# lithium0003/findtextCenterNet

Hardware: AMD Instinct MI355X
Metric: 768x768 images/s (detector fwd+NMS) (higher is better)
Workload: dtype bf16; 1 GPU; BASELINE configs[1]: batch=8/GPU synthetic 768x768x3 uniform-noise tiles, full EfficientNetV2-XL detector forward + NMS + GPU peak decode/100-d gather; global_batch=8, tile=768x768x3, weights=deterministic seed 0 (random-init), parallelism=dp1

## Files before the change

### findtextcenternet_amd/csrc/mbconv_slice.hip

```cpp
#include "conv_igemm_impl.h"

namespace {
using namespace convimpl;

struct MbsP {
    const void* x;
    const void* we;
    const float* be;
    const float* wd;
    const float* bd;
    void* out;
    float* sums;
    const float* w1;
    float* hpart;
    int B, H, W, K, C, S;
    int R, nb;
    int kblock;
    unsigned img_bytes;
    float inv_hw;
    unsigned long long* tl;
};

constexpr int MS_NT = 512;
constexpr int MS_MAXPX = 576;
constexpr int MS_XS = MS_MAXPX * 64;
constexpr int MS_NSTAGE = 3;
constexpr int MS_MAXSLOT = 601;
constexpr int MS_R = 6;
template <int NCT> struct MsGeom {
    static constexpr int CC = NCT * 32;
    static constexpr int CQN = CC / 4;
    static constexpr int NPL = MS_NT / CQN;
    static constexpr int STAGE = MS_XS + CC * 64;
    static constexpr int PITCH = CC * 2 + 8;
    static constexpr int IMG = MS_MAXSLOT * PITCH, RING = MS_NSTAGE * STAGE;
    static constexpr int CONST = ((IMG > RING ? IMG : RING) + 15) / 16 * 16;
    static constexpr int LDS = CONST + 10 * CC * 4;
    static constexpr int NPIECE = 36 + CC / 16;
    static constexpr int NW6 = NPIECE - 40;
    static_assert(LDS <= 160 * 1024 && NPIECE > 40 && NPIECE <= 48, "");
};

__device__ __forceinline__ f32x4 mfma16x16(bf16x8 a, bf16x8 b, f32x4 c) { return __builtin_amdgcn_mfma_f32_16x16x32_bf16(a, b, c, 0, 0, 0); }
__device__ __forceinline__ f32x4 mfma16x16(f16x8 a, f16x8 b, f32x4 c) { return __builtin_amdgcn_mfma_f32_16x16x32_f16(a, b, c, 0, 0, 0); }

template <typename T> struct Raw4;
template <> struct Raw4<__bf16> { using type = bf16x4; };
template <> struct Raw4<_Float16> { using type = f16x4; };
template <typename V> __device__ __forceinline__ f32x4 widen4(V v) { return f32x4{(float)v[0], (float)v[1], (float)v[2], (float)v[3]}; }
template <int N> struct MsInt { static constexpr int value = N; };

constexpr int MS_GENERAL = 0, MS_MAP24 = 1, MS_BAND48 = 2;

template <typename T, int FORM, int NCT = 4>
__global__ __launch_bounds__(MS_NT, 2) void mbconv_slice_kernel(const MbsP p) {
    constexpr bool FAST = FORM == MS_MAP24;
    using GM = MsGeom<NCT>;
    constexpr int MS_CC = GM::CC, MS_STAGE = GM::STAGE, MS_PITCH = GM::PITCH, MS_CONST = GM::CONST, CQN = GM::CQN, NPL = GM::NPL;
    extern __shared__ __attribute__((aligned(16))) unsigned char smem_raw[];
    const int t = threadIdx.x;
    const int lane = t & 63;
    const int wave = __builtin_amdgcn_readfirstlane(t >> 6);
    const int l15 = lane & 15, lq = lane >> 4;
    const int bid = blockIdx.x;
    const int b = bid % p.B;
    const int rest = bid / p.B;
    const int band = FAST ? 0 : rest % p.nb, sl = FAST ? rest : rest / p.nb;
    const int c0 = sl * MS_CC;
    const int W = FAST ? 24 : FORM == MS_BAND48 ? 48 : p.W;
    const int y0 = FAST ? 0 : band * p.R, y1 = FAST ? 24 : min(p.H, y0 + p.R);
    const int ylo = FAST ? 0 : max(0, y0 - 1), yhi = FAST ? 24 : min(p.H, y1 + 1);
    const int H = yhi - ylo;
    const int M = H * W;
    const int W1 = W + 1;
    const int Mfull = p.H * W;

    const unsigned xbase = (unsigned)ylo * W * (p.kblock ? 64u : (unsigned)p.K * 2u);
    const __amdgpu_buffer_rsrc_t rx = __builtin_amdgcn_make_buffer_rsrc(const_cast<char*>(static_cast<const char*>(p.x) + (size_t)b * p.img_bytes + xbase), 0,
                                                                        p.img_bytes - xbase, 0x00020000);
    const __amdgpu_buffer_rsrc_t rwe = __builtin_amdgcn_make_buffer_rsrc(const_cast<char*>(static_cast<const char*>(p.we) + (size_t)c0 * p.K * 2), 0,
                                                                         (unsigned)(MS_CC * p.K * 2), 0x00020000);

    constexpr int NLMAX = 6;
    int s_off[NLMAX];
#pragma unroll
    for (int i = 0; i < NLMAX; ++i) {
        const int q = (i * 8 + wave) * 64 + lane;
        const bool isx = q < MS_MAXPX * 4;
        const int row = isx ? (q >> 2) : ((q - MS_MAXPX * 4) >> 2);
        const int kc = (q & 3) ^ (((row >> 3) & 1) * 3);
        const int rowb = (isx && p.kblock) ? 64 : p.K * 2;
        s_off[i] = (!isx || row < M) ? row * rowb + kc * 16 : OOB;
    }
    const int xstep = p.kblock ? Mfull * 64 : 64;
    auto issue_piece = [&](int i, int step, int bufoff) {
        const int q0 = (i * 8 + wave) * 64;
        if (i < 5 || wave < GM::NW6) {
            lds_void_t* dst = (lds_void_t*)(smem_raw + bufoff + q0 * 16);
            if (q0 < MS_MAXPX * 4) glds16(rx, dst, s_off[i], step * xstep);
            else glds16(rwe, dst, s_off[i], step * 64);
        }
    };

    const int chw = wave & 1, pg = wave >> 1;
    f32x4 acc[NCT][9];
#pragma unroll
    for (int i = 0; i < NCT; ++i) {
        const f32x4 bi = *reinterpret_cast<const f32x4*>(p.be + c0 + chw * (MS_CC / 2) + i * 16 + 4 * lq);
#pragma unroll
        for (int j = 0; j < 9; ++j) acc[i][j] = bi;
    }
    if (t < 10 * CQN) {
        const int row = t / CQN, ch = (t - row * CQN) * 4;
        const f32x4 v = *reinterpret_cast<const f32x4*>(row < 9 ? p.wd + (long)row * p.C + c0 + ch : p.bd + c0 + ch);
        *reinterpret_cast<f32x4*>(smem_raw + MS_CONST + t * 16) = v;
    }

    using FragT = typename Frag<T>::type;
    const int swz = ((lq ^ (((l15 >> 3) & 1) * 3)) << 4);
    const int offA = MS_XS + (chw * (MS_CC / 2) + l15) * 64 + swz;
    const int offB = (pg * 144 + l15) * 64 + swz;
    const int nk = p.K >> 5;
    const bool tl_on = p.tl && t == 0;
    unsigned long long* tl = p.tl + (size_t)blockIdx.x * 32;
    if (tl_on) tl[0] = __builtin_amdgcn_s_memtime();
#pragma unroll
    for (int i = 0; i < NLMAX; ++i) issue_piece(i, 0, 0);
    if (nk > 1) {
#pragma unroll
        for (int i = 0; i < NLMAX; ++i) issue_piece(i, 1, MS_STAGE);
    }
    int cur_off = 0, iss_off = 2 * MS_STAGE;
    unsigned long long tw = 0, tw0 = 0;
    for (int it = 0; it < nk; ++it) {
        const unsigned long long ta = tl_on ? __builtin_amdgcn_s_memtime() : 0;
        if (it + 1 >= nk) wait_vmcnt<0>();
        else if (wave < GM::NW6) wait_vmcnt<6>();
        else wait_vmcnt<5>();
        wg_barrier();
        if (tl_on) { const unsigned long long d = __builtin_amdgcn_s_memtime() - ta; tw += d; if (it == 0) tw0 = d; if (it < 24) tl[8 + it] = ta; }
        const unsigned char* base = smem_raw + cur_off;
        const bool more = it + 2 < nk;
        FragT af[NCT];
#pragma unroll
        for (int i = 0; i < NCT; ++i) af[i] = *reinterpret_cast<const FragT*>(base + offA + i * 1024);
        FragT bq[3];
#pragma unroll
        for (int j = 0; j < 3; ++j) bq[j] = *reinterpret_cast<const FragT*>(base + offB + j * 1024);
#pragma unroll
        for (int j = 0; j < 9; ++j) {
            const FragT bcur = bq[j % 3];
            if (j + 3 < 9) bq[j % 3] = *reinterpret_cast<const FragT*>(base + offB + (j + 3) * 1024);
#pragma unroll
            for (int i = 0; i < NCT; ++i) acc[i][j] = mfma16x16(af[i], bcur, acc[i][j]);
            constexpr int piece_after[9] = {0, 1, -1, 2, 3, -1, 4, 5, -1};
            if (piece_after[j] >= 0 && more) issue_piece(piece_after[j], it + 2, iss_off);
            __builtin_amdgcn_sched_barrier(0);
        }
        iss_off = iss_off + MS_STAGE == MS_NSTAGE * MS_STAGE ? 0 : iss_off + MS_STAGE;
        cur_off = cur_off + MS_STAGE == MS_NSTAGE * MS_STAGE ? 0 : cur_off + MS_STAGE;
    }
    wg_barrier();
    if (tl_on) { tl[1] = __builtin_amdgcn_s_memtime(); tl[5] = tw; tl[6] = tw0; }

    for (int idx = t; idx < (H + 1) * CQN; idx += MS_NT) {
        const u32x2 z = {0u, 0u};
        *reinterpret_cast<u32x2*>(smem_raw + ((idx / CQN) * W1) * MS_PITCH + (idx % CQN) * 8) = z;
    }
#pragma unroll
    for (int j = 0; j < 9; ++j) {
        const int m = pg * 144 + j * 16 + l15;
        if (m < M) {
            const int y = m / W;
            unsigned char* row = smem_raw + (m + y + 1) * MS_PITCH + (chw * (MS_CC / 2) + 4 * lq) * 2;
#pragma unroll
            for (int i = 0; i < NCT; ++i) store4<T>(reinterpret_cast<T*>(row + i * 32), act_silu_fast4(acc[i][j]));
        }
    }
    __syncthreads();
    if (tl_on) tl[2] = __builtin_amdgcn_s_memtime();

    const int pl = t / CQN, cq = t - pl * CQN;
    const bool dw_on = pl < NPL;
    const int c = c0 + cq * 4;
    constexpr int NU = (FTC_MBHEAD_MAX_SQUEEZE + NPL - 1) / NPL;
    f32x4 w1r[NU];
    auto load_w1 = [&]() {
#pragma unroll
        for (int i = 0; i < NU; ++i) {
            const int su = pl + NPL * i;
            w1r[i] = (dw_on && su < p.S) ? *reinterpret_cast<const f32x4*>(p.w1 + (size_t)su * p.C + c) : f32x4{0.f, 0.f, 0.f, 0.f};
        }
    };
    if (p.hpart) load_w1();
    f32x4 wv[9];
#pragma unroll
    for (int k = 0; k < 9; ++k) wv[k] = *reinterpret_cast<const f32x4*>(smem_raw + MS_CONST + k * (MS_CC * 4) + cq * 16);
    const f32x4 bv = *reinterpret_cast<const f32x4*>(smem_raw + MS_CONST + 9 * (MS_CC * 4) + cq * 16);
    const int yo = y0 - ylo, yend = y1 - ylo;
    const int nsr = (yend - yo + MS_R - 1) / MS_R;
    const int nstrips = nsr * W;
    f32x4 sum = {0.f, 0.f, 0.f, 0.f};
    T* outp = reinterpret_cast<T*>(p.out) + ((size_t)b * Mfull + (size_t)ylo * W) * p.C + c;
    const unsigned char* zslot = smem_raw + cq * 8;
    using R4 = typename Raw4<T>::type;
    auto run_strips = [&](auto nr_c, int s, const int lim) __attribute__((always_inline)) {
        constexpr int NR = decltype(nr_c)::value;
        for (; s < lim; s += NPL) {
            const int sr = s / W, x = s - sr * W;
            const int oy0 = yo + sr * MS_R;
            const unsigned char* base0 = smem_raw + ((oy0 - 1) * W1 + x) * MS_PITCH + cq * 8;
            const unsigned char* base1 = base0 + 7 * W1 * MS_PITCH;
            R4 win[(NR + 2) * 3];
#pragma unroll
            for (int r = 0; r < NR + 2; ++r) {
                const bool rok = r == 0 ? oy0 > 0 : r == NR + 1 ? oy0 + NR < H : true;
                const unsigned char* rp = (r < 7 ? base0 + r * W1 * MS_PITCH : base1 + (r - 7) * W1 * MS_PITCH);
#pragma unroll
                for (int s2 = 0; s2 < 3; ++s2) win[r * 3 + s2] = *reinterpret_cast<const R4*>(rok ? rp + s2 * MS_PITCH : zslot);
            }
            f32x4 a[NR];
#pragma unroll
            for (int oo = 0; oo < NR; ++oo) a[oo] = bv;
#pragma unroll
            for (int r = 0; r < NR + 2; ++r) {
                f32x4 xin[3];
#pragma unroll
                for (int s2 = 0; s2 < 3; ++s2) xin[s2] = widen4(win[r * 3 + s2]);
#pragma unroll
                for (int oo = 0; oo < NR; ++oo) {
                    const int kr = r - oo;
                    if (kr >= 0 && kr < 3) {
#pragma unroll
                        for (int s2 = 0; s2 < 3; ++s2)
#pragma unroll
                            for (int e = 0; e < 4; ++e) a[oo][e] = fmaf(wv[kr * 3 + s2][e], xin[s2][e], a[oo][e]);
                    }
                }
            }
#pragma unroll
            for (int oo = 0; oo < NR; ++oo) {
                a[oo] = act_silu_fast4(a[oo]);
                store4<T>(outp + ((oy0 + oo) * W + x) * p.C, a[oo]);
                sum += a[oo];
            }
        }
        return s;
    };
    {
        int s = dw_on ? pl : nstrips;
        if constexpr (FAST) {
            for (; s < nstrips; s += NPL) {
                const int sr = s / W, x = s - sr * W;
                const int oy0 = yo + sr * MS_R;
                const unsigned char* base0 = smem_raw + ((oy0 - 1) * W1 + x) * MS_PITCH + cq * 8;
                const unsigned char* base1 = base0 + 7 * W1 * MS_PITCH;
                f32x4 a[MS_R];
#pragma unroll
                for (int oo = 0; oo < MS_R; ++oo) a[oo] = bv;
#pragma unroll
                for (int r = 0; r < MS_R + 2; ++r) {
                    const bool rok = r == 0 ? oy0 > 0 : r == MS_R + 1 ? oy0 + MS_R < 24 : true;
                    const unsigned char* rp = (r < 7 ? base0 + r * W1 * MS_PITCH : base1 + (r - 7) * W1 * MS_PITCH);
                    f32x4 xin[3];
#pragma unroll
                    for (int s2 = 0; s2 < 3; ++s2) xin[s2] = load4<T>(reinterpret_cast<const T*>(rok ? rp + s2 * MS_PITCH : zslot));
#pragma unroll
                    for (int oo = 0; oo < MS_R; ++oo) {
                        const int kr = r - oo;
                        if (kr >= 0 && kr < 3) {
#pragma unroll
                            for (int s2 = 0; s2 < 3; ++s2)
#pragma unroll
                                for (int e = 0; e < 4; ++e) a[oo][e] = fmaf(wv[kr * 3 + s2][e], xin[s2][e], a[oo][e]);
                        }
                    }
                }
#pragma unroll
                for (int oo = 0; oo < MS_R; ++oo) {
                    a[oo] = act_silu_fast4(a[oo]);
                    store4<T>(outp + ((oy0 + oo) * W + x) * p.C, a[oo]);
                    sum += a[oo];
                }
            }
        } else {
            const int hl = (yend - yo) - (nsr - 1) * MS_R;
            s = run_strips(MsInt<MS_R>{}, s, hl == MS_R ? nstrips : nstrips - W);
            switch (hl) {
                case 1: run_strips(MsInt<1>{}, s, nstrips); break;
                case 2: run_strips(MsInt<2>{}, s, nstrips); break;
                case 3: run_strips(MsInt<3>{}, s, nstrips); break;
                case 4: run_strips(MsInt<4>{}, s, nstrips); break;
                case 5: run_strips(MsInt<5>{}, s, nstrips); break;
                default: break;
            }
        }
    }
    if (tl_on) tl[3] = __builtin_amdgcn_s_memtime();

    __syncthreads();
    constexpr int NRED = NCT == 4 ? 8 : NPL;
    float* red = reinterpret_cast<float*>(smem_raw);
    float* lmean = red + NRED * MS_CC;
    if constexpr (NCT == 4) {
        f32x4 v = sum;
#pragma unroll
        for (int e = 0; e < 4; ++e) v[e] += __shfl_xor(v[e], 32, 64);
        if (lane < 32) *reinterpret_cast<f32x4*>(red + wave * MS_CC + lane * 4) = v;
    } else {
        if (dw_on) *reinterpret_cast<f32x4*>(red + pl * MS_CC + cq * 4) = sum;
    }
    __syncthreads();
    if (t < MS_CC) {
        float tot = 0.f;
#pragma unroll
        for (int w8 = 0; w8 < NRED; ++w8) tot += red[w8 * MS_CC + t];
        p.sums[((size_t)b * p.nb + band) * p.C + c0 + t] = tot;
        lmean[t] = tot * p.inv_hw;
    }
    if (p.hpart) {
        __syncthreads();
        float* fcb = lmean + MS_CC;
        const f32x4 m4 = *reinterpret_cast<const f32x4*>(lmean + (dw_on ? cq : 0) * 4);
#pragma unroll
        for (int i = 0; i < NU; ++i) {
            const f32x4 pr = w1r[i] * m4;
            const int su = pl + NPL * i;
            if (dw_on && su < p.S) fcb[su * (CQN + 1) + cq] = (pr[0] + pr[1]) + (pr[2] + pr[3]);
        }
        __syncthreads();
        if (t < p.S) {
            float d = 0.f;
#pragma unroll
            for (int q = 0; q < CQN; ++q) d += fcb[t * (CQN + 1) + q];
            float* dst = p.hpart + (((size_t)b * p.nb + band) * (p.C / MS_CC) + sl) * p.S + t;
            *dst = d;
        }
    }
    if (tl_on) tl[4] = __builtin_amdgcn_s_memtime();
}

}

static int mbhead_rows(const ftc_op& o) { return o.aux1 > 0 ? (o.aux1 + 2 < o.H ? o.aux1 + 2 : o.H) : o.H; }

bool ftc_mbhead_legal(const ftc_op& o) {
    const int rows = mbhead_rows(o);
    const bool x3 = o.in_dtype == FTC_F32 && (o.flags & FTC_FLAG_SPLIT16);
    const int slice = ftc_mbhead_slice(o);
    if (x3 ? slice != FTC_MBHEAD_SLICE_F32 : (slice != 128 && slice != 96)) return false;
    return (ftc_is16(o.in_dtype) || x3) && o.in_dtype == o.out_dtype && o.in_dtype == o.w_dtype && o.stride == 1 && o.ksize == 3 && o.Ho == o.H &&
           o.Wo == o.W && o.aux1 >= 0 && rows * o.W <= MS_MAXPX && rows * (o.W + 1) + 1 <= MS_MAXSLOT && o.Cout > 0 &&
           o.Cout % slice == 0 && o.Cin > 0 && o.Cin % 32 == 0;
}

int ftc_mbhead_slice(const ftc_op& o) { return o.Cout_total > 0 ? o.Cout_total : (o.in_dtype == FTC_F32 ? FTC_MBHEAD_SLICE_F32 : FTC_MBHEAD_SLICE); }

int ftc_mbhead_bands(const ftc_op& o) { return o.aux1 > 0 ? (o.H + o.aux1 - 1) / o.aux1 : 1; }

int ftc_mbhead_band_rows(int H, int W) {
    if (H * W <= MS_MAXPX && H * (W + 1) + 1 <= MS_MAXSLOT) return 0;
    int r = MS_MAXPX / W;
    while (r > 2 && r * (W + 1) + 1 > MS_MAXSLOT) --r;
    return r - 2 > 0 ? r - 2 : -1;
}

bool ftc_mbhead_whole_map(const ftc_op& o) { return o.H == 24 && o.W == 24 && ftc_mbhead_bands(o) == 1 && !(o.flags & 0x100); }

static bool ftc_mbhead_band48(const ftc_op& o) { return o.aux1 > 0 && o.W == 48 && !(o.flags & 0x100); }

hipError_t launch_mbhead_x3(const OpArgs& a, hipStream_t s);

hipError_t launch_mbhead(const OpArgs& a, hipStream_t s) {
    const ftc_op& o = *a.op;
    if (!ftc_mbhead_legal(o)) return hipErrorInvalidValue;
    if (o.in_dtype == FTC_F32) return launch_mbhead_x3(a, s);
    MbsP p;
    p.x = a.in; p.we = a.w2; p.be = a.bias2; p.wd = static_cast<const float*>(a.w); p.bd = a.bias; p.out = a.out; p.sums = a.aux;
    p.w1 = a.scale; p.hpart = a.scale ? static_cast<float*>(a.out2) : nullptr;
    p.B = o.B; p.H = o.H; p.W = o.W; p.K = o.Cin; p.C = o.Cout; p.S = o.aux0;
    p.kblock = (o.flags & FTC_FLAG_KBLOCK32) ? 1 : 0;
    p.R = o.aux1 > 0 ? o.aux1 : o.H; p.nb = ftc_mbhead_bands(o);
    p.img_bytes = (unsigned)((long)o.H * o.W * o.Cin * 2);
    p.inv_hw = 1.0f / (float)(o.H * o.W);
    p.tl = (o.flags & 0x1000) ? reinterpret_cast<unsigned long long*>(const_cast<void*>(a.in2)) : nullptr;
    const int slice = ftc_mbhead_slice(o);
    const int nblk = o.B * p.nb * (o.Cout / slice);
    const int form = ftc_mbhead_whole_map(o) ? MS_MAP24 : ftc_mbhead_band48(o) ? MS_BAND48 : MS_GENERAL;
    hipError_t e = hipSuccess;
#define MBS_LAUNCH(T, F, N) do {                                                                                                   \
        if ((e = ftc_allow_dyn_lds(reinterpret_cast<const void*>(mbconv_slice_kernel<T, F, N>), MsGeom<N>::LDS)) == hipSuccess) \
            hipLaunchKernelGGL((mbconv_slice_kernel<T, F, N>), dim3(nblk), dim3(MS_NT), MsGeom<N>::LDS, s, p);                  \
    } while (0)
#define MBS_PICK(T, N) do { if (form == MS_MAP24) MBS_LAUNCH(T, MS_MAP24, N); else if (form == MS_BAND48) MBS_LAUNCH(T, MS_BAND48, N); \
                            else MBS_LAUNCH(T, MS_GENERAL, N); } while (0)
    if (o.in_dtype == FTC_F16) { if (slice == 96) MBS_PICK(_Float16, 3); else MBS_PICK(_Float16, 4); }
    else { if (slice == 96) MBS_PICK(__bf16, 3); else MBS_PICK(__bf16, 4); }
#undef MBS_PICK
#undef MBS_LAUNCH
    return e != hipSuccess ? e : hipGetLastError();
}
```

Baseline: 726.4 images/s.

## Issue all global-to-LDS loads from waves 0-3 only and add timing probe variant

Moves all async global-to-LDS piece loads in the mbconv slice K-loop onto waves 0-3, which now issue up to eleven pieces each per stage, while waves 4-7 only compute and wait at the barrier. The intent is to take DMA-issue and vmcnt-wait overhead off half the waves so their MFMA stream runs uninterrupted. The cost is a heavier issue load on the issuer waves and a longer wait window before each barrier. It also adds a flag-gated timing template (TLW) that records per-wave wait, barrier and DMA times plus SIMD ids, which is off by default.

```diff
diff --git a/findtextcenternet_amd/csrc/mbconv_slice.hip b/findtextcenternet_amd/csrc/mbconv_slice.hip
--- a/findtextcenternet_amd/csrc/mbconv_slice.hip
+++ b/findtextcenternet_amd/csrc/mbconv_slice.hip
@@ -49,10 +49,12 @@
 template <> struct Raw4<_Float16> { using type = f16x4; };
 template <typename V> __device__ __forceinline__ f32x4 widen4(V v) { return f32x4{(float)v[0], (float)v[1], (float)v[2], (float)v[3]}; }
 template <int N> struct MsInt { static constexpr int value = N; };
+template <bool V> struct MsBool { static constexpr bool value = V; };
+template <int N, int...> struct MsFirst { static constexpr int value = N; };
 
 constexpr int MS_GENERAL = 0, MS_MAP24 = 1, MS_BAND48 = 2;
 
-template <typename T, int FORM, int NCT = 4>
+template <typename T, int FORM, int NCT = 4, int TLW = -1>
 __global__ __launch_bounds__(MS_NT, 2) void mbconv_slice_kernel(const MbsP p) {
     constexpr bool FAST = FORM == MS_MAP24;
     using GM = MsGeom<NCT>;
@@ -81,11 +83,13 @@
     const __amdgpu_buffer_rsrc_t rwe = __builtin_amdgcn_make_buffer_rsrc(const_cast<char*>(static_cast<const char*>(p.we) + (size_t)c0 * p.K * 2), 0,
                                                                          (unsigned)(MS_CC * p.K * 2), 0x00020000);
 
-    constexpr int NLMAX = 6;
+    constexpr int NLMAX = 11;
+    static_assert(GM::NW6 <= 4, "waves 4-7 have five pieces each: numbers 6-10 of their SIMD partner");
+    const bool issuer = wave < 4;
     int s_off[NLMAX];
 #pragma unroll
     for (int i = 0; i < NLMAX; ++i) {
-        const int q = (i * 8 + wave) * 64 + lane;
+        const int q = ((i < 6 ? i : i - 6) * 8 + (i < 6 ? wave : wave + 4)) * 64 + lane;
         const bool isx = q < MS_MAXPX * 4;
         const int row = isx ? (q >> 2) : ((q - MS_MAXPX * 4) >> 2);
         const int kc = (q & 3) ^ (((row >> 3) & 1) * 3);
@@ -94,8 +98,9 @@
     }
     const int xstep = p.kblock ? Mfull * 64 : 64;
     auto issue_piece = [&](int i, int step, int bufoff) {
-        const int q0 = (i * 8 + wave) * 64;
-        if (i < 5 || wave < GM::NW6) {
+        const int ii = i < 6 ? i : i - 6, wv = i < 6 ? wave : wave + 4;
+        const int q0 = (ii * 8 + wv) * 64;
+        if (issuer && (ii < 5 || wv < GM::NW6)) {
             lds_void_t* dst = (lds_void_t*)(smem_raw + bufoff + q0 * 16);
             if (q0 < MS_MAXPX * 4) glds16(rx, dst, s_off[i], step * xstep);
             else glds16(rwe, dst, s_off[i], step * 64);
@@ -121,7 +126,9 @@
     const int offA = MS_XS + (chw * (MS_CC / 2) + l15) * 64 + swz;
     const int offB = (pg * 144 + l15) * 64 + swz;
     const int nk = p.K >> 5;
-    const bool tl_on = p.tl && t == 0;
+    constexpr bool DET = TLW >= 0;
+    const bool tl_on = p.tl && t == (DET ? TLW * 64 : 0);
+    const bool det_w = DET && wave == TLW;
     unsigned long long* tl = p.tl + (size_t)blockIdx.x * 32;
     if (tl_on) tl[0] = __builtin_amdgcn_s_memtime();
 #pragma unroll
@@ -132,34 +139,58 @@
     }
     int cur_off = 0, iss_off = 2 * MS_STAGE;
     unsigned long long tw = 0, tw0 = 0;
-    for (int it = 0; it < nk; ++it) {
-        const unsigned long long ta = tl_on ? __builtin_amdgcn_s_memtime() : 0;
-        if (it + 1 >= nk) wait_vmcnt<0>();
-        else if (wave < GM::NW6) wait_vmcnt<6>();
-        else wait_vmcnt<5>();
-        wg_barrier();
-        if (tl_on) { const unsigned long long d = __builtin_amdgcn_s_memtime() - ta; tw += d; if (it == 0) tw0 = d; if (it < 24) tl[8 + it] = ta; }
-        const unsigned char* base = smem_raw + cur_off;
-        const bool more = it + 2 < nk;
-        FragT af[NCT];
-#pragma unroll
-        for (int i = 0; i < NCT; ++i) af[i] = *reinterpret_cast<const FragT*>(base + offA + i * 1024);
-        FragT bq[3];
-#pragma unroll
-        for (int j = 0; j < 3; ++j) bq[j] = *reinterpret_cast<const FragT*>(base + offB + j * 1024);
-#pragma unroll
-        for (int j = 0; j < 9; ++j) {
-            const FragT bcur = bq[j % 3];
-            if (j + 3 < 9) bq[j % 3] = *reinterpret_cast<const FragT*>(base + offB + (j + 3) * 1024);
-#pragma unroll
-            for (int i = 0; i < NCT; ++i) acc[i][j] = mfma16x16(af[i], bcur, acc[i][j]);
-            constexpr int piece_after[9] = {0, 1, -1, 2, 3, -1, 4, 5, -1};
-            if (piece_after[j] >= 0 && more) issue_piece(piece_after[j], it + 2, iss_off);
-            __builtin_amdgcn_sched_barrier(0);
-        }
-        iss_off = iss_off + MS_STAGE == MS_NSTAGE * MS_STAGE ? 0 : iss_off + MS_STAGE;
-        cur_off = cur_off + MS_STAGE == MS_NSTAGE * MS_STAGE ? 0 : cur_off + MS_STAGE;
-    }
+    auto sat16 = [](unsigned long long v) { return v > 0xffffull ? 0xffffull : v; };
+    auto kloop = [&](auto issuer_c) __attribute__((always_inline)) {
+        constexpr bool ISSUER = decltype(issuer_c)::value;
+        for (int it = 0; it < nk; ++it) {
+            const unsigned long long ta = (tl_on || det_w) ? __builtin_amdgcn_s_memtime() : 0;
+            unsigned long long d_vm = 0, d_bar = 0, d_first = 0, d_dma = 0;
+            if constexpr (ISSUER) {
+                if (it + 1 >= nk) wait_vmcnt<0>();
+                else if (wave < GM::NW6) wait_vmcnt<11>();
+                else wait_vmcnt<10>();
+            }
+            const unsigned long long tb = det_w ? __builtin_amdgcn_s_memtime() : 0;
+            wg_barrier();
+            if (tl_on) { const unsigned long long d = __builtin_amdgcn_s_memtime() - ta; tw += d; if (it == 0) tw0 = d; if (!DET && it < 24) tl[8 + it] = ta; }
+            if constexpr (DET) { if (det_w) { const unsigned long long tc = __builtin_amdgcn_s_memtime(); d_vm = tb - ta; d_bar = tc - tb; d_first = tc; } }
+            const unsigned char* base = smem_raw + cur_off;
+            const bool more = it + 2 < nk;
+            FragT af[NCT];
+#pragma unroll
+            for (int i = 0; i < NCT; ++i) af[i] = *reinterpret_cast<const FragT*>(base + offA + i * 1024);
+            FragT bq[3];
+#pragma unroll
+            for (int j = 0; j < 3; ++j) bq[j] = *reinterpret_cast<const FragT*>(base + offB + j * 1024);
+            if constexpr (DET) {
+                if (det_w) { asm volatile("s_waitcnt lgkmcnt(0)" ::: "memory"); d_first = __builtin_amdgcn_s_memtime() - d_first; }
+                __builtin_amdgcn_sched_barrier(0);
+            }
+#pragma unroll
+            for (int j = 0; j < 9; ++j) {
+                const FragT bcur = bq[j % 3];
+                if (j + 3 < 9) bq[j % 3] = *reinterpret_cast<const FragT*>(base + offB + (j + 3) * 1024);
+#pragma unroll
+                for (int i = 0; i < NCT; ++i) acc[i][j] = mfma16x16(af[i], bcur, acc[i][j]);
+                if constexpr (ISSUER) {
+                    if (more) {
+                        const unsigned long long t0 = det_w ? __builtin_amdgcn_s_memtime() : 0;
+                        issue_piece(j, it + 2, iss_off);
+                        if (j == 2) issue_piece(9, it + 2, iss_off);
+                        if (j == 5) issue_piece(10, it + 2, iss_off);
+                        if constexpr (DET) { if (det_w) d_dma += __builtin_amdgcn_s_memtime() - t0; }
+                    }
+                }
+                __builtin_amdgcn_sched_barrier(0);
+            }
+            if constexpr (DET) {
+                if (tl_on && it < 24) tl[8 + it] = sat16(d_vm) | sat16(d_bar) << 16 | sat16(d_first) << 32 | sat16(d_dma) << 48;
+            }
+            iss_off = iss_off + MS_STAGE == MS_NSTAGE * MS_STAGE ? 0 : iss_off + MS_STAGE;
+            cur_off = cur_off + MS_STAGE == MS_NSTAGE * MS_STAGE ? 0 : cur_off + MS_STAGE;
+        }
+    };
+    if (issuer) kloop(MsBool<true>{}); else kloop(MsBool<false>{});
     wg_barrier();
     if (tl_on) { tl[1] = __builtin_amdgcn_s_memtime(); tl[5] = tw; tl[6] = tw0; }
 
@@ -338,6 +369,17 @@
         }
     }
     if (tl_on) tl[4] = __builtin_amdgcn_s_memtime();
+    if constexpr (DET) {
+        __syncthreads();
+        unsigned* sid = reinterpret_cast<unsigned*>(smem_raw + MS_CONST);
+        if (lane == 0) sid[wave] = __builtin_amdgcn_s_getreg(4 | (4 << 6) | (1 << 11)) | 8u;
+        __syncthreads();
+        if (tl_on) {
+            unsigned long long v = 0;
+            for (int w = 0; w < MS_NT / 64; ++w) v |= (unsigned long long)sid[w] << (4 * w);
+            tl[7] = v;
+        }
+    }
 }
 
 }
@@ -388,12 +430,18 @@
     const int nblk = o.B * p.nb * (o.Cout / slice);
     const int form = ftc_mbhead_whole_map(o) ? MS_MAP24 : ftc_mbhead_band48(o) ? MS_BAND48 : MS_GENERAL;
     hipError_t e = hipSuccess;
-#define MBS_LAUNCH(T, F, N) do {                                                                                                   \
-        if ((e = ftc_allow_dyn_lds(reinterpret_cast<const void*>(mbconv_slice_kernel<T, F, N>), MsGeom<N>::LDS)) == hipSuccess) \
-            hipLaunchKernelGGL((mbconv_slice_kernel<T, F, N>), dim3(nblk), dim3(MS_NT), MsGeom<N>::LDS, s, p);                  \
+#define MBS_LAUNCH(T, F, ...) do {                                                                                                           \
+        constexpr int lds = MsGeom<MsFirst<__VA_ARGS__>::value>::LDS;                                                                         \
+        if ((e = ftc_allow_dyn_lds(reinterpret_cast<const void*>(mbconv_slice_kernel<T, F, __VA_ARGS__>), lds)) == hipSuccess)               \
+            hipLaunchKernelGGL((mbconv_slice_kernel<T, F, __VA_ARGS__>), dim3(nblk), dim3(MS_NT), lds, s, p);                                \
     } while (0)
 #define MBS_PICK(T, N) do { if (form == MS_MAP24) MBS_LAUNCH(T, MS_MAP24, N); else if (form == MS_BAND48) MBS_LAUNCH(T, MS_BAND48, N); \
                             else MBS_LAUNCH(T, MS_GENERAL, N); } while (0)
+    if (o.flags & 0x2000) {
+        if (!p.tl || o.in_dtype != FTC_BF16 || slice != 128 || form == MS_GENERAL) return hipErrorInvalidValue;
+        if (o.flags & 0x4000) { if (form == MS_MAP24) MBS_LAUNCH(__bf16, MS_MAP24, 4, 4); else MBS_LAUNCH(__bf16, MS_BAND48, 4, 4); }
+        else { if (form == MS_MAP24) MBS_LAUNCH(__bf16, MS_MAP24, 4, 0); else MBS_LAUNCH(__bf16, MS_BAND48, 4, 0); }
+    } else
     if (o.in_dtype == FTC_F16) { if (slice == 96) MBS_PICK(_Float16, 3); else MBS_PICK(_Float16, 4); }
     else { if (slice == 96) MBS_PICK(__bf16, 3); else MBS_PICK(__bf16, 4); }
 #undef MBS_PICK
```

New measurement: 731.2 images/s, median of 6. No clear change (+0.7%).
